# damien911224/ZeroShotVideoClassification

Hardware: AMD Instinct MI355X
Metric: clips/sec (fwd+bwd+step) R(2+1)D-18 16x112x112 bs=22/GPU (higher is better)
Workload: dtype f32

## Files before the change

### zeroshotvideoclassification_amd/csrc/conv_wgrad.hip

```cpp
#include <hip/hip_runtime.h>
#include <stdint.h>
#include <stdlib.h>
#include "conv_params.h"
#include "knobs.h"

namespace zsv {

typedef float f32x2 __attribute__((ext_vector_type(2)));

struct WgradParams {
    int M;
    int Cin, Cpad, nblk;
    int taps, kHW, kW;
    int Kp;
    int P;
    int oS, oHW, oW;
    Magic m_oS, m_oHW, m_oW;
    int gT, gH, gW, gS, gHW, gCS;
    int sT, sH, sW, pT, pH, pW;
    int chunks_per_slice;
    unsigned x_bytes, dy_bytes;
};

template <int TM, int TN, int WGM, int WGN, bool AV4, int BP, bool TWOTAP>
__global__ __launch_bounds__(256, (BP == 16 ? 3 : 2)) void conv_wgrad_kernel(WgradParams prm, const float* __restrict__ X,
                                                         const float* __restrict__ DY,
                                                         float* __restrict__ OUT, int tiles_m, int tiles_mn) {
    constexpr int BM = 16 * TM * WGM;
    constexpr int BN = 16 * TN * WGN;
    constexpr int LDK = BP + 2;
    constexpr int NBLK = BN / 16;
    constexpr int RW = 64 / BP;
    constexpr int RPP = 4 * RW;
    constexpr int PB = 16 / RPP;
    constexpr int BPASS = NBLK * PB;
    constexpr int AQ = BP / 4;
    constexpr int ARP = 256 / AQ;
    constexpr int APASS = AV4 ? (BM + ARP - 1) / ARP : BM / RPP;
    constexpr unsigned OOB = 0xFFFFFFFFu;
    static_assert(WGM * WGN == 4, "4 waves");
    static_assert(BM % RPP == 0 || AV4, "tile rows must be a multiple of the staging pass");

    __shared__ __attribute__((aligned(16))) float As[2][BM * LDK];
    __shared__ float Bs[2][BN * LDK];

    const int tid = threadIdx.x;
    const int lane = tid & 63;
    const int wave = sgpr(tid >> 6);
    const int wm0 = (wave / WGN) * (16 * TM);
    const int wn0 = (wave % WGN) * (16 * TN);
    const int lin = xcd_tile(gridDim.x, blockIdx.x);
    const int tile = lin % tiles_mn;
    const int slice = lin / tiles_mn;
    const int m0 = (tile % tiles_m) * BM;
    const int n0 = (tile / tiles_m) * BN;

    const __amdgpu_buffer_rsrc_t x_rsrc = __builtin_amdgcn_make_buffer_rsrc(const_cast<float*>(X), 0, prm.x_bytes, 0x00020000);
// ... 157 lines not shown
    const int frag_k = lane >> 4;
    const int frag_r = lane & 15;
    constexpr int NG = BP / 8;
    for (int ch = chunk_begin; ch < chunk_end; ++ch) {
        const int cur = (ch - chunk_begin) & 1;
        if (ch + 1 < chunk_end) store_chunk(cur ^ 1);
        const int lchunk = min(ch + 2, chunk_end - 1);
        const float* as = &As[cur][0];
        const float* bs = &Bs[cur][0];
        float a[2][2][TM], b[2][2][TN];
        auto fetch = [&](int g, int slot) {
#pragma unroll
            for (int kk = 0; kk < 2; ++kk) {
#pragma unroll
                for (int i = 0; i < TM; ++i) a[slot][kk][i] = as[(wm0 + 16 * i + frag_r) * LDK + (2 * g + kk) * 4 + frag_k];
#pragma unroll
                for (int j = 0; j < TN; ++j) b[slot][kk][j] = bs[(wn0 + 16 * j + frag_r) * LDK + (2 * g + kk) * 4 + frag_k];
            }
        };
        fetch(0, 0);
#pragma unroll
        for (int g = 0; g < NG; ++g) {
            if (g + 1 < NG) fetch(g + 1, (g + 1) & 1);
            __builtin_amdgcn_sched_barrier(0);
            load_part(lchunk, g, NG);
#pragma unroll
            for (int kk = 0; kk < 2; ++kk)
#pragma unroll
                for (int i = 0; i < TM; ++i)
#pragma unroll
                    for (int j = 0; j < TN; ++j)
                        acc[i][j] = __builtin_amdgcn_mfma_f32_16x16x4f32(a[g & 1][kk][i], b[g & 1][kk][j], acc[i][j], 0, 0, 0);
            __builtin_amdgcn_sched_barrier(0);
        }
        __syncthreads();
    }

    float* out = OUT + (size_t)slice * prm.M * prm.Kp;
#pragma unroll
    for (int j = 0; j < TN; ++j) {
        const int k = n0 + wn0 + 16 * j + frag_r;
        if (k >= prm.Kp) continue;
#pragma unroll
        for (int i = 0; i < TM; ++i) {
#pragma unroll
            for (int r = 0; r < 4; ++r) {
                const int m = m0 + wm0 + 16 * i + 4 * frag_k + r;
                if (m < prm.M) out[(size_t)m * prm.Kp + k] = acc[i][j][r];
            }
        }
    }
}

__global__ __launch_bounds__(256) void slab_sum_kernel(const float* __restrict__ slabs, float* __restrict__ out,
                                                       int M, int Cin, int taps, int Cpad, int slices) {
    __shared__ float part[8][32];
    const size_t slab = (size_t)M * taps * Cpad;
    const int e = threadIdx.x & 31, g = threadIdx.x >> 5;
    for (size_t j0 = (size_t)blockIdx.x * 32; j0 < slab; j0 += (size_t)gridDim.x * 32) {
        const size_t j = j0 + e;
        const int ci = (int)(j % Cpad);
        const bool live = j < slab && ci < Cin;
        float s = 0.f;
        if (live) {
            const float* src = slabs + j;
            int k = g;
            for (; k + 24 < slices; k += 32) {
                const float v0 = src[(size_t)k * slab], v1 = src[(size_t)(k + 8) * slab];
                const float v2 = src[(size_t)(k + 16) * slab], v3 = src[(size_t)(k + 24) * slab];
                s += v0; s += v1; s += v2; s += v3;
            }
            for (; k < slices; k += 8) s += src[(size_t)k * slab];
        }
        part[g][e] = s;
        __syncthreads();
        if (g == 0 && live) {
            float t = part[0][e];
#pragma unroll
            for (int q = 1; q < 8; ++q) t += part[q][e];
            const size_t r = j / Cpad;
            const int tap = (int)(r % taps);
            const int co = (int)(r / taps);
            out[((size_t)co * Cin + ci) * taps + tap] = t;
        }
        __syncthreads();
    }
}

__global__ __launch_bounds__(256) void slab_sum_rows_kernel(const float* __restrict__ slabs, float* __restrict__ out,
                                                            int M, int Cin, int taps, int Cpad, int slices) {
    extern __shared__ __attribute__((aligned(16))) float row[];
    const int co = blockIdx.x;
    const int len = taps * Cpad;
    const size_t slab = (size_t)M * len;
    const float* src = slabs + (size_t)co * len;
    for (int i = 4 * (int)threadIdx.x; i < len; i += 1024) {
        f32x4 t = *reinterpret_cast<const f32x4*>(src + i);
        int k = 1;
        for (; k + 2 < slices; k += 3) {
            const f32x4 v0 = *reinterpret_cast<const f32x4*>(src + (size_t)k * slab + i);
            const f32x4 v1 = *reinterpret_cast<const f32x4*>(src + (size_t)(k + 1) * slab + i);
            const f32x4 v2 = *reinterpret_cast<const f32x4*>(src + (size_t)(k + 2) * slab + i);
            t += v0; t += v1; t += v2;
        }
        for (; k < slices; ++k) t += *reinterpret_cast<const f32x4*>(src + (size_t)k * slab + i);
        *reinterpret_cast<f32x4*>(row + i) = t;
    }
    __syncthreads();
    float* dst = out + (size_t)co * Cin * taps;
    const int n = Cin * taps;
    for (int o = (int)threadIdx.x; o < n; o += 256) {
        const int ci = o / taps, tap = o - ci * taps;
        dst[o] = row[tap * Cpad + ci];
    }
}

int slab_sum(const float* slabs, float* dw, int M, int Cin, int taps, int Cpad, int slices, hipStream_t stream) {
    const size_t row_bytes = (size_t)taps * Cpad * sizeof(float);
    if (slices <= 32 && (long)M * slices <= 16384 && row_bytes <= 64 * 1024 && (reinterpret_cast<uintptr_t>(slabs) & 15) == 0 && !ZSV_KNOB(NO_SLAB_SUM_ROWS)) {
        static const hipError_t attr = hipFuncSetAttribute((const void*)slab_sum_rows_kernel, hipFuncAttributeMaxDynamicSharedMemorySize, 64 * 1024);
        if (attr != hipSuccess) return ZSV_E_LAUNCH;
        hipLaunchKernelGGL(slab_sum_rows_kernel, dim3((unsigned)M), dim3(256), row_bytes, stream, slabs, dw, M, Cin, taps, Cpad, slices);
        return hipGetLastError() == hipSuccess ? ZSV_OK : ZSV_E_LAUNCH;
    }
    const long n = (long)M * taps * Cpad;
    long blocks = (n + 31) / 32;
    if (blocks > 8192) blocks = 8192;
    hipLaunchKernelGGL(slab_sum_kernel, dim3((unsigned)blocks), dim3(256), 0, stream, slabs, dw, M, Cin, taps, Cpad, slices);
    return hipGetLastError() == hipSuccess ? ZSV_OK : ZSV_E_LAUNCH;
}

static int wgrad_bp() { return 32; }

__global__ __launch_bounds__(256) void t2_fold_kernel(const float* __restrict__ dw2, float* __restrict__ dw, int Cout, int Cin) {
    const long n = (long)Cout * Cin;
    for (long i = (long)blockIdx.x * 256 + threadIdx.x; i < n; i += (long)gridDim.x * 256) {
        const long co = i / Cin, c = i - co * Cin;
        const float* r0 = dw2 + (2 * co) * (2L * Cin) + 2 * c;
        const float* r1 = r0 + 2L * Cin;
        const f32x2 a = *reinterpret_cast<const f32x2*>(r0), b = *reinterpret_cast<const f32x2*>(r1);
        dw[3 * i] = b[0];
        dw[3 * i + 1] = a[0] + b[1];
        dw[3 * i + 2] = a[1];
    }
}

struct WgradPlan {
    int cfg;
    int bm, bn;
    int tiles_m, tiles_n, slices, chunks_per_slice;
    int Cpad, nblk, Kp;
};

static double wgrad_slices(long tiles, long chunks, int bp, int bm, int bn, long& slices) {
    const long lds_bytes = (long)(bm + bn) * 34 * 4 * 2;
    long per_cu = (160L * 1024) / lds_bytes;
    if (per_cu > 4) per_cu = 4;
    if (per_cu < 1) per_cu = 1;
    const long resident = 256L * per_cu;
    long max_slices = (chunks * bp + 511) / 512;
    if (max_slices < 1) max_slices = 1;
    if (max_slices > 1024) max_slices = 1024;
    slices = 1;
    double best_eff = -1.0;
    for (long s = 1; s <= max_slices && tiles * s <= 4 * resident + tiles; ++s) {
        const long wgs = tiles * s;
        const long rounds = (wgs + resident - 1) / resident;
        const double eff = (double)wgs / (double)(rounds * resident) - 0.02 * (double)wgs / (double)resident;
        if (eff > best_eff + 1e-9) { best_eff = eff; slices = s; }
    }
    return best_eff;
}

static WgradPlan wgrad_plan(const zsv_conv_desc* d) {
    WgradPlan pl;
    const int M = d->Cout;
    const int taps = d->kT * d->kH * d->kW;
    pl.nblk = (d->Cin + 15) / 16;
    pl.Cpad = pl.nblk * 16;
    pl.Kp = taps * pl.Cpad;
    const long P = (long)d->N * d->To * d->Ho * d->Wo;
    const int bp = wgrad_bp();
// ... 205 lines not shown
```

### zeroshotvideoclassification_amd/csrc/conv_wgrad_tring.hip

```cpp
#include <hip/hip_runtime.h>
#include <stdlib.h>

#include "conv_params.h"
#include "zsv_common.h"
#include "zsv_hip.h"
#include "knobs.h"

namespace zsv {

typedef __attribute__((address_space(3))) void* lds_ptr_t;

struct WgradTringParams {
    int M, Cin;
    int S, HW, T, nseg;
    int chunks_total, chunks_per_slice;
    int slices;
    unsigned x_bytes, dy_bytes;
    int tiles_m, tiles_mn;
    const float* pre_coef;
    int pre_pitch;
};

__device__ __forceinline__ int tring_swz(int row) { return ((row >> 2) & 1) << 1; }

template <int TM, bool PRE = false>
__global__ __launch_bounds__(256, 3) void conv_wgrad_tring_kernel(WgradTringParams prm, const float* __restrict__ X,
                                                                  const float* __restrict__ DY, float* __restrict__ OUT) {
#if defined(__HIP_DEVICE_COMPILE__)
    constexpr int BM = 16 * TM;
    constexpr int NAW = (TM + 3) / 4;
    constexpr int A_BYTES = TM * 1024;
    constexpr int RING_AT = 2 * A_BYTES;
    constexpr unsigned OOB = 0xFFFFFFF0u;
    extern __shared__ __attribute__((aligned(16))) unsigned char lds[];

    const int tid = threadIdx.x, lane = tid & 63;
    const int wave = __builtin_amdgcn_readfirstlane(tid >> 6);
    const int lid = xcd_tile(gridDim.x, blockIdx.x);
    const int tile = lid % prm.tiles_mn, slice = lid / prm.tiles_mn;
    const int m0 = (tile % prm.tiles_m) * BM, co0 = (tile / prm.tiles_m) * 64;
    const int c0 = slice * prm.chunks_per_slice;
    const int nq = min(prm.chunks_per_slice, prm.chunks_total - c0);
    if (nq <= 0) return;

    const __amdgpu_buffer_rsrc_t rs_x = __builtin_amdgcn_make_buffer_rsrc(const_cast<float*>(X), 0, prm.x_bytes, 0x00020000);
    const __amdgpu_buffer_rsrc_t rs_dy = __builtin_amdgcn_make_buffer_rsrc(const_cast<float*>(DY), 0, prm.dy_bytes, 0x00020000);

    const int prow = lane >> 2, srcslot = ((lane & 3) ^ tring_swz(prow)) * 4;
    int a_off[NAW];
#pragma unroll
    for (int k = 0; k < NAW; ++k) {
        const int pa = wave + 4 * k;
        const int ci = m0 + pa * 16 + prow;
        a_off[k] = (pa < TM && ci < prm.Cin) ? 4 * (ci * prm.S + srcslot) : -1;
    }
    const int co_l = co0 + wave * 16 + prow;
    const int b_off = co_l < prm.M ? 4 * (co_l * prm.S + srcslot) : -1;

    auto issue_x = [&](int buf, int n_img, int t, int seg) {
// ... 232 lines not shown
            const int sl = i & 1;
            if (i + 1 < TM) {
#pragma unroll
                for (int j = 0; j < 4; ++j) xf[sl ^ 1][j] = *reinterpret_cast<const f32x4*>(xs[j] + (i + 1) * 1024);
            }
            f32x4 d0 = xf[sl][0], d1 = xf[sl][1], d2 = xf[sl][2], d3 = xf[sl][3];
            if constexpr (PRE) {
#pragma unroll
                for (int s = 0; s < 4; ++s) {
                    d0[s] = fmaxf(__fmaf_rn(d0[s], pre_sc[i], pre_sh[i]), 0.f);
                    d1[s] = fmaxf(__fmaf_rn(d1[s], pre_sc[i], pre_sh[i]), 0.f);
                    d2[s] = fmaxf(__fmaf_rn(d2[s], pre_sc[i], pre_sh[i]), 0.f);
                    d3[s] = fmaxf(__fmaf_rn(d3[s], pre_sc[i], pre_sh[i]), 0.f);
                }
            }
            if (zero_d0) d0 = f32x4{0.f, 0.f, 0.f, 0.f};
            if (zero_d3) d3 = f32x4{0.f, 0.f, 0.f, 0.f};
            const f32x4 v0 = d0 - d2, v1 = d1 + d2, v2 = d2 - d1, v3 = d1 - d3;
            __builtin_amdgcn_sched_barrier(0);
            __builtin_amdgcn_s_setprio(1);
#pragma unroll
            for (int s = 0; s < 4; ++s) {
                acc[i][0] = __builtin_amdgcn_mfma_f32_16x16x4f32(v0[s], y0[s], acc[i][0], 0, 0, 0);
                acc[i][1] = __builtin_amdgcn_mfma_f32_16x16x4f32(v1[s], bsum[s], acc[i][1], 0, 0, 0);
                acc[i][2] = __builtin_amdgcn_mfma_f32_16x16x4f32(v2[s], bdif[s], acc[i][2], 0, 0, 0);
                acc[i][3] = __builtin_amdgcn_mfma_f32_16x16x4f32(v3[s], y1[s], acc[i][3], 0, 0, 0);
            }
            __builtin_amdgcn_s_setprio(0);
            __builtin_amdgcn_sched_barrier(0);
        }
        asm volatile("s_waitcnt vmcnt(0)" ::: "memory");
        __syncthreads();
        head = ring(head, 2);
        if (ntp == 0) job += prm.slices;
        tp = ntp; seg = nseg_; n_img = nn;
    }

    const int co = co0 + wave * 16 + r16;
    if (co < prm.M) {
        float* out = OUT + (size_t)slice * 4 * prm.Cin * prm.M;
#pragma unroll
        for (int p = 0; p < 4; ++p)
#pragma unroll
            for (int i = 0; i < TM; ++i)
#pragma unroll
                for (int r = 0; r < 4; ++r) {
                    const int ci = m0 + 16 * i + 4 * g + r;
                    if (ci < prm.Cin) out[((size_t)p * prm.Cin + ci) * prm.M + co] = acc[i][p][r];
                }
    }
#endif
}

__global__ __launch_bounds__(256) void wgrad_twino_sum_kernel(const float* __restrict__ slabs, float* __restrict__ dw, int M,
                                                              int Cin, int slices) {
    __shared__ float part[8][4][32];
    const size_t plane = (size_t)Cin * M;
    const int e = threadIdx.x & 31, grp = threadIdx.x >> 5;
    for (size_t j0 = (size_t)blockIdx.x * 32; j0 < plane; j0 += (size_t)gridDim.x * 32) {
        const size_t j = j0 + e;
        const bool live = j < plane;
        float s[4] = {0.f, 0.f, 0.f, 0.f};
        if (live) {
            int k = grp;
            for (; k + 24 < slices; k += 32) {
                float v[4][4];
#pragma unroll
                for (int u = 0; u < 4; ++u)
#pragma unroll
                    for (int p = 0; p < 4; ++p) v[u][p] = slabs[((size_t)(k + 8 * u) * 4 + p) * plane + j];
#pragma unroll
                for (int u = 0; u < 4; ++u)
#pragma unroll
                    for (int p = 0; p < 4; ++p) s[p] += v[u][p];
            }
            for (; k < slices; k += 8)
#pragma unroll
                for (int p = 0; p < 4; ++p) s[p] += slabs[((size_t)k * 4 + p) * plane + j];
        }
#pragma unroll
        for (int p = 0; p < 4; ++p) part[grp][p][e] = s[p];
        __syncthreads();
        if (grp == 0 && live) {
            float Mv[4];
#pragma unroll
            for (int p = 0; p < 4; ++p) {
                float t = part[0][p][e];
#pragma unroll
                for (int q = 1; q < 8; ++q) t += part[q][p][e];
                Mv[p] = t;
            }
            const int co = (int)(j % M), ci = (int)(j / M);
            float* o = dw + ((size_t)co * Cin + ci) * 3;
            const float h = 0.5f * (Mv[1] + Mv[2]);
            o[0] = Mv[0] + h;
            o[1] = 0.5f * (Mv[1] - Mv[2]);
            o[2] = h - Mv[3];
        }
        __syncthreads();
    }
}

__global__ __launch_bounds__(256) void wgrad_tring_sum_kernel(const float* __restrict__ slabs, float* __restrict__ dw, int M,
                                                              int Cin, int slices) {
    __shared__ float part[8][32];
    const size_t slab = (size_t)Cin * 3 * M;
    const int e = threadIdx.x & 31, grp = threadIdx.x >> 5;
    for (size_t j0 = (size_t)blockIdx.x * 32; j0 < slab; j0 += (size_t)gridDim.x * 32) {
        const size_t j = j0 + e;
        const bool live = j < slab;
        float s = 0.f;
        if (live) {
            int k = grp;
            for (; k + 24 < slices; k += 32) {
                const float v0 = slabs[(size_t)k * slab + j], v1 = slabs[(size_t)(k + 8) * slab + j];
                const float v2 = slabs[(size_t)(k + 16) * slab + j], v3 = slabs[(size_t)(k + 24) * slab + j];
                s += v0; s += v1; s += v2; s += v3;
            }
            for (; k < slices; k += 8) s += slabs[(size_t)k * slab + j];
        }
        part[grp][e] = s;
        __syncthreads();
        if (grp == 0 && live) {
            float v = part[0][e];
#pragma unroll
            for (int q = 1; q < 8; ++q) v += part[q][e];
            const int co = (int)(j % M);
            const size_t rr = j / M;
            const int kt = (int)(rr % 3), ci = (int)(rr / 3);
            dw[((size_t)co * Cin + ci) * 3 + kt] = v;
        }
        __syncthreads();
    }
}

struct WgradTringPlan {
    int tm, tiles_m, tiles_n, slices, chunks_per_slice;
};

static WgradTringPlan wgrad_tring_plan(const zsv_conv_desc* d) {
    WgradTringPlan pl;
    const int C = d->Cin;
    const int p9 = (C + 143) / 144 * 144, p8 = (C + 127) / 128 * 128;
    pl.tm = p9 <= p8 ? 9 : 8;
    const int bm = 16 * pl.tm;
    pl.tiles_m = (C + bm - 1) / bm;
    pl.tiles_n = (d->Cout + 63) / 64;
    const long chunks = (long)d->N * d->Ti * (d->Hi * d->Wi / 16);
    const long tiles = (long)pl.tiles_m * pl.tiles_n;
    long resident = pl.tm == 9 ? 512 : 768;
    if (const char* e = ZSV_KNOB(WGRAD_TRING_RESIDENT)) resident = atol(e) > 0 ? atol(e) : resident;
    const double t_mfma = 2.0 * (double)(pl.tiles_m * bm) * (double)(pl.tiles_n * 192) * (double)chunks * 16.0 / 1.1e14;
    const double t_slice = 2.0 * (double)C * 3.0 * d->Cout * sizeof(float) / 6.0e12;
    long max_sl = chunks / 32;
    if (max_sl < 1) max_sl = 1;
    if (max_sl > 4096) max_sl = 4096;
    long sl = 1;
    double best = 1e300;
    for (long c = 1; c <= max_sl; ++c) {
        const long wgs = tiles * c, rounds = (wgs + resident - 1) / resident;
        const double cost = t_mfma * (double)(rounds * resident) / (double)wgs + t_slice * (double)c;
        if (cost < best * 0.999) { best = cost; sl = c; }
    }
    if (const char* e = ZSV_KNOB(WGRAD_TRING_SLICES)) sl = atol(e) > 0 ? atol(e) : 1;
    if (sl > chunks) sl = chunks;
    pl.chunks_per_slice = (int)((chunks + sl - 1) / sl);
    pl.slices = (int)((chunks + pl.chunks_per_slice - 1) / pl.chunks_per_slice);
    return pl;
}

bool wgrad_tring_applicable(const zsv_conv_desc* d, const float* x, const float* dy) {
    if (ZSV_KNOB(NO_WGRAD_TRING)) return false;
    if (d->kT != 3 || d->kH != 1 || d->kW != 1 || d->sT != 1 || d->sH != 1 || d->sW != 1 || d->pT != 1 || d->pH != 0 || d->pW != 0)
        return false;
    if (d->Ti % 4 != 0 || (d->Hi * d->Wi) % 16 != 0) return false;
    if (d->Cout < 32) return false;
    const long S = (long)d->Ti * d->Hi * d->Wi;
    if ((long)d->N * d->Cin * S >= (1L << 29) || (long)d->N * d->Cout * S >= (1L << 29)) return false;
    const int C = d->Cin, p9 = (C + 143) / 144 * 144, p8 = (C + 127) / 128 * 128, pc = p9 <= p8 ? p9 : p8;
    if (pc * 10 > C * 13) return false;
    const int pm = (d->Cout + 63) / 64 * 64;
    if (pm * 10 > d->Cout * 13) return false;
    if ((long)d->N * S < 16384) return false;
    if (x != nullptr && ((reinterpret_cast<uintptr_t>(x) | reinterpret_cast<uintptr_t>(dy)) & 15) != 0) return false;
    return true;
}

// ... 43 lines not shown

template <int TM, bool PRE>
static int wgrad_twino_launch(const WgradTringParams& p, int slices, hipStream_t stream, const float* x, const float* dy,
                              float* out) {
    constexpr int LDS_BYTES = 6 * TM * 1024 + 4 * 4096;
    static const hipError_t attr = hipFuncSetAttribute((const void*)conv_wgrad_twino_kernel<TM, PRE>,
                                                       hipFuncAttributeMaxDynamicSharedMemorySize, LDS_BYTES);
    if (attr != hipSuccess) return ZSV_E_LAUNCH;
    hipLaunchKernelGGL((conv_wgrad_twino_kernel<TM, PRE>), dim3((unsigned)(p.tiles_mn * slices)), dim3(256), LDS_BYTES, stream, p, x,
                       dy, out);
    return launch_status();
}

template <int TM, bool PRE>
static int wgrad_tring_launch(const WgradTringParams& p, int slices, hipStream_t stream, const float* x, const float* dy,
                              float* out) {
    constexpr int LDS_BYTES = 2 * TM * 1024 + 4 * 4096;
    static const hipError_t attr = hipFuncSetAttribute((const void*)conv_wgrad_tring_kernel<TM, PRE>,
                                                       hipFuncAttributeMaxDynamicSharedMemorySize, LDS_BYTES);
    if (attr != hipSuccess) return ZSV_E_LAUNCH;
    hipLaunchKernelGGL((conv_wgrad_tring_kernel<TM, PRE>), dim3((unsigned)(p.tiles_mn * slices)), dim3(256), LDS_BYTES, stream, p, x,
                       dy, out);
    return launch_status();
}

int wgrad_tring(const zsv_conv_desc* d, const float* x, const float* dy, float* dw, void* workspace, size_t workspace_bytes,
                hipStream_t stream) {
    return wgrad_tring_pre(d, x, nullptr, 0, dy, dw, workspace, workspace_bytes, stream);
}

int wgrad_tring_pre(const zsv_conv_desc* d, const float* x, const float* pre_coef, int pre_pitch, const float* dy, float* dw,
                    void* workspace, size_t workspace_bytes, hipStream_t stream) {
    const bool twino = wgrad_twino_shape(d);
    const WgradTringPlan pl = twino ? wgrad_twino_plan(d) : wgrad_tring_plan(d);
    if (!workspace || workspace_bytes < wgrad_tring_workspace_bytes(d)) return ZSV_E_WORKSPACE;
    WgradTringParams p;
    p.M = d->Cout; p.Cin = d->Cin;
    p.S = d->Ti * d->Hi * d->Wi; p.HW = d->Hi * d->Wi; p.T = d->Ti; p.nseg = p.HW / 16;
    p.chunks_total = d->N * (twino ? p.T / 2 : p.T) * p.nseg;
    p.chunks_per_slice = pl.chunks_per_slice;
    p.slices = pl.slices;
    p.x_bytes = 4u * (unsigned)((long)d->N * d->Cin * p.S);
    p.dy_bytes = 4u * (unsigned)((long)d->N * d->Cout * p.S);
    p.tiles_m = pl.tiles_m; p.tiles_mn = pl.tiles_m * pl.tiles_n;
    p.pre_coef = pre_coef; p.pre_pitch = pre_pitch;
    float* slabs = (float*)workspace;
    int st;
    if (twino) {
        if (pre_coef) st = pl.tm == 9 ? wgrad_twino_launch<9, true>(p, pl.slices, stream, x, dy, slabs)
                                      : wgrad_twino_launch<8, true>(p, pl.slices, stream, x, dy, slabs);
        else st = pl.tm == 9 ? wgrad_twino_launch<9, false>(p, pl.slices, stream, x, dy, slabs)
                             : wgrad_twino_launch<8, false>(p, pl.slices, stream, x, dy, slabs);
        if (st) return st;
        const long n = (long)d->Cin * d->Cout;
        long blocks = (n + 31) / 32;
        if (blocks > 8192) blocks = 8192;
        hipLaunchKernelGGL(wgrad_twino_sum_kernel, dim3((unsigned)blocks), dim3(256), 0, stream, (const float*)slabs, dw, d->Cout,
                           d->Cin, pl.slices);
        return launch_status();
    }
    if (pre_coef) st = pl.tm == 9 ? wgrad_tring_launch<9, true>(p, pl.slices, stream, x, dy, slabs)
                                  : wgrad_tring_launch<8, true>(p, pl.slices, stream, x, dy, slabs);
    else st = pl.tm == 9 ? wgrad_tring_launch<9, false>(p, pl.slices, stream, x, dy, slabs)
                         : wgrad_tring_launch<8, false>(p, pl.slices, stream, x, dy, slabs);
    if (st) return st;
    const long n = (long)d->Cin * 3 * d->Cout;
    long blocks = (n + 31) / 32;
    if (blocks > 8192) blocks = 8192;
    hipLaunchKernelGGL(wgrad_tring_sum_kernel, dim3((unsigned)blocks), dim3(256), 0, stream, (const float*)slabs, dw, d->Cout,
                       d->Cin, pl.slices);
    return launch_status();
}

}
```

### zeroshotvideoclassification_amd/csrc/conv_wgrad_wino.hip

```cpp
#include <hip/hip_runtime.h>
#include <stdlib.h>

#include "conv_params.h"
#include "zsv_common.h"
#include "zsv_hip.h"
#include "knobs.h"

namespace zsv {

typedef __attribute__((address_space(3))) void* lds_ptr_t;
typedef unsigned u32x4w __attribute__((ext_vector_type(4)));

struct WgradWinoParams {
    int M, Cin, Cpad, R, Kp;
    int S, HW, W, kT;
    int chunks_total, chunks_per_slice, cpc;
    unsigned x_bytes, dy_bytes, vm_bytes;
    int tiles_m, tiles_mn;
};

template <int TM, int TN, bool EDGE>
__global__ __launch_bounds__(256, 2) void conv_wgrad_wino_kernel(WgradWinoParams prm, const float* __restrict__ X,
                                                                 const float* __restrict__ DY,
                                                                 const unsigned* __restrict__ VM, float* __restrict__ OUT) {
#if defined(__HIP_DEVICE_COMPILE__)
    constexpr int BM = 16 * TM;
    constexpr int LDA = 36, LDB = 44;
    constexpr int NA_TOT = (BM * 9 + 63) / 64;
    constexpr int BN = 64 * TN;
    constexpr int NB_TOT = 11 * TN;
    constexpr int NA = (NA_TOT + 3) / 4, NB = (NB_TOT + 3) / 4;
    constexpr int A_BYTES = NA_TOT * 1024, B_BYTES = NB_TOT * 1024;
    constexpr int VM_AT = A_BYTES + B_BYTES;
    constexpr int STAGE = VM_AT + 1024;
    constexpr unsigned OOB = 0xFFFFFFF0u;
    extern __shared__ __attribute__((aligned(16))) unsigned char lds[];

    const int tid = threadIdx.x, lane = tid & 63;
    const int wave = __builtin_amdgcn_readfirstlane(tid >> 6);
    const int lid = xcd_tile(gridDim.x, blockIdx.x);
    const int tile = lid % prm.tiles_mn, slice = lid / prm.tiles_mn;
    const int m0 = (tile % prm.tiles_m) * BM, n0 = (tile / prm.tiles_m) * BN;
    const int c0 = slice * prm.chunks_per_slice;
    const int nq = min(prm.chunks_per_slice, prm.chunks_total - c0);
    const int cpc = prm.cpc;
    int n_img = c0 / cpc;
    int p_local = (c0 - n_img * cpc) * 32;

    const __amdgpu_buffer_rsrc_t rs_dy = __builtin_amdgcn_make_buffer_rsrc(const_cast<float*>(DY), 0, prm.dy_bytes, 0x00020000);
    const __amdgpu_buffer_rsrc_t rs_x = __builtin_amdgcn_make_buffer_rsrc(const_cast<float*>(X), 0, prm.x_bytes, 0x00020000);
    const __amdgpu_buffer_rsrc_t rs_vm = __builtin_amdgcn_make_buffer_rsrc(const_cast<unsigned*>(VM), 0, prm.vm_bytes, 0x00020000);

    int a_off[NA], a_vox[NA];
#pragma unroll
    for (int k = 0; k < NA; ++k) {
        const int id = 64 * (wave + 4 * k) + lane;
        const int row = id / 9, pc = id - row * 9;
        const bool ok = row < BM && m0 + row < prm.M && pc < 8;
        a_off[k] = ok ? 4 * ((m0 + row) * prm.S + 4 * pc) : -1;
// ... 270 lines not shown
                V[4][s] = fmaf(-2.f, t5, t6);
                V[5][s] = fmaf(4.f, d1, fmaf(-5.f, d3, d5));
            }
        }
#pragma unroll
        for (int i = 0; i < TMX; ++i) {
            if (TMA != TMB && i >= tmw) break;
            const int sl = i & 1;
            if (i + 1 < TMX) {
                ar[sl ^ 1][0] = *reinterpret_cast<const f32x4*>(st + a_frag + (i + 1) * 16 * LDA * 4);
                ar[sl ^ 1][1] = *reinterpret_cast<const f32x4*>(st + a_frag + (i + 1) * 16 * LDA * 4 + 16);
            }
            float Av[6][2];
#pragma unroll
            for (int s = 0; s < 2; ++s) {
                const float y0 = ar[sl][s][0], y1 = ar[sl][s][1], y2 = ar[sl][s][2], y3 = ar[sl][s][3];
                const float e = y0 + y2, o = y1 + y3, e4 = fmaf(4.f, y2, y0), q = fmaf(4.f, y3, y1);
                Av[0][s] = y0; Av[1][s] = e + o; Av[2][s] = e - o;
                Av[3][s] = fmaf(2.f, q, e4); Av[4][s] = fmaf(-2.f, q, e4); Av[5][s] = y3;
            }
            __builtin_amdgcn_sched_barrier(0);
            __builtin_amdgcn_s_setprio(1);
#pragma unroll
            for (int s = 0; s < 2; ++s)
#pragma unroll
                for (int p = 0; p < 6; ++p)
                    acc[p][i] = __builtin_amdgcn_mfma_f32_16x16x4f32(Av[p][s], V[p][s], acc[p][i], 0, 0, 0);
            __builtin_amdgcn_s_setprio(0);
            __builtin_amdgcn_sched_barrier(0);
        }
        asm volatile("s_waitcnt vmcnt(0)" ::: "memory");
        __syncthreads();
    }

    float* out = OUT + (size_t)slice * 6 * prm.M * prm.Kp;
    const int n = n0 + 16 * cw + r16;
    if (n < prm.Kp) {
#pragma unroll
        for (int p = 0; p < 6; ++p)
#pragma unroll
            for (int i = 0; i < TMX; ++i) {
                if (TMA != TMB && i >= tmw) break;
#pragma unroll
                for (int r = 0; r < 4; ++r) {
                    const int m = m0 + 16 * (i0 + i) + 4 * g + r;
                    if (m < prm.M) out[((size_t)p * prm.M + m) * prm.Kp + n] = acc[p][i][r];
                }
            }
    }
#endif
}

template <int PTS>
__global__ __launch_bounds__(256) void wgrad_wino_sum_kernel(const float* __restrict__ slabs, float* __restrict__ dw, int M,
                                                             int Cin, int R, int Cpad, int slices) {
    __shared__ float part[8][PTS][32];
    const size_t plane = (size_t)M * R * Cpad;
    const int e = threadIdx.x & 31, grp = threadIdx.x >> 5;
    for (size_t j0 = (size_t)blockIdx.x * 32; j0 < plane; j0 += (size_t)gridDim.x * 32) {
        const size_t j = j0 + e;
        const int ci = (int)(j % Cpad);
        const bool live = j < plane && ci < Cin;
        float s[PTS];
#pragma unroll
        for (int p = 0; p < PTS; ++p) s[p] = 0.f;
        if (live) {
            int k = grp;
            for (; k + 8 < slices; k += 16) {
                float v[2][PTS];
#pragma unroll
                for (int u = 0; u < 2; ++u)
#pragma unroll
                    for (int p = 0; p < PTS; ++p) v[u][p] = slabs[((size_t)(k + 8 * u) * PTS + p) * plane + j];
#pragma unroll
                for (int u = 0; u < 2; ++u)
#pragma unroll
                    for (int p = 0; p < PTS; ++p) s[p] += v[u][p];
            }
            for (; k < slices; k += 8)
#pragma unroll
                for (int p = 0; p < PTS; ++p) s[p] += slabs[((size_t)k * PTS + p) * plane + j];
        }
#pragma unroll
        for (int p = 0; p < PTS; ++p) part[grp][p][e] = s[p];
        __syncthreads();
        if (grp == 0 && live) {
            float Mv[PTS];
#pragma unroll
            for (int p = 0; p < PTS; ++p) {
                float t = part[0][p][e];
#pragma unroll
                for (int q = 1; q < 8; ++q) t += part[q][p][e];
                Mv[p] = t;
            }
            const size_t rr = j / Cpad;
            const int r = (int)(rr % R), co = (int)(rr / R);
            float* o = dw + (((size_t)co * Cin + ci) * R + r) * 3;
            if constexpr (PTS == 4) {
                const float h = 0.5f * (Mv[1] + Mv[2]);
                o[0] = Mv[0] + h;
                o[1] = 0.5f * (Mv[1] - Mv[2]);
                o[2] = h - Mv[3];
            } else {
                const float s12 = Mv[1] + Mv[2], d12 = Mv[2] - Mv[1], s34 = Mv[3] + Mv[4], d34 = Mv[3] - Mv[4];
                o[0] = 0.25f * Mv[0] - s12 * (1.f / 6.f) + s34 * (1.f / 24.f);
                o[1] = d12 * (1.f / 6.f) + d34 * (1.f / 12.f);
                o[2] = Mv[5] - s12 * (1.f / 6.f) + s34 * (1.f / 6.f);
            }
        }
        __syncthreads();
    }
}

struct WgradWinoPlan {
    int tm, tn, tiles_m, tiles_n, slices, chunks_per_slice, Cpad, Kp;
};

static WgradWinoPlan wgrad_wino_plan(const zsv_conv_desc* d) {
    WgradWinoPlan pl;
    const int M = d->Cout;
    pl.Cpad = (d->Cin + 15) / 16 * 16;
    pl.Kp = 3 * d->kT * pl.Cpad;
    const int p9 = (M + 143) / 144 * 144, p8 = (M + 127) / 128 * 128;
    pl.tm = M <= 64 ? 4 : (p9 <= p8 ? 9 : 8);
    pl.tn = pl.tm == 4 ? 2 : 1;
    const int bm = 16 * pl.tm, bn = 64 * pl.tn;
    pl.tiles_m = (M + bm - 1) / bm;
    pl.tiles_n = (pl.Kp + bn - 1) / bn;
    const long chunks = (long)d->N * (((long)d->Ti * d->Hi * d->Wi + 31) / 32);
    const long tiles = (long)pl.tiles_m * pl.tiles_n, resident = 512;
    const double voxels = (double)chunks * 32.0;
    const double t_mfma = 4.0 * (double)(pl.tiles_m * bm) * (double)(pl.tiles_n * bn) * voxels / 1.1e14;
    const double t_slice = 2.0 * 4.0 * (double)M * pl.Kp * sizeof(float) / 6.0e12;
    long max_sl = chunks / 24;
    if (max_sl < 1) max_sl = 1;
    if (max_sl > 4096) max_sl = 4096;
    long sl = 1;
    double best = 1e300;
    for (long c = 1; c <= max_sl; ++c) {
        const long wgs = tiles * c, rounds = (wgs + resident - 1) / resident;
        const double cost = t_mfma * (double)(rounds * resident) / (double)wgs + t_slice * (double)c;
        if (cost < best * 0.999) { best = cost; sl = c; }
    }
    if (const char* e = ZSV_KNOB(WGRAD_WINO_SLICES)) sl = atol(e);
    if (sl < 1) sl = 1;
    if (sl > chunks) sl = chunks;
    pl.chunks_per_slice = (int)((chunks + sl - 1) / sl);
    pl.slices = (int)((chunks + pl.chunks_per_slice - 1) / pl.chunks_per_slice);
    return pl;
}

bool wgrad_wino_applicable(const zsv_conv_desc* d, const float* x, const float* dy) {
    if (ZSV_KNOB(NO_WINO) || ZSV_KNOB(NO_WGRAD_WINO)) return false;
    if ((d->kT != 1 && d->kT != 3) || d->kH != 3 || d->kW != 3 || d->sT != 1 || d->sH != 1 || d->sW != 1 || d->pT != d->kT / 2 ||
        d->pH != 1 || d->pW != 1)
        return false;
    if (d->Wi % 2 != 0 || d->Cin < 16) return false;
    const long S = (long)d->Ti * d->Hi * d->Wi;
    if (S % 4 != 0) return false;
    if ((long)d->N * d->Cin * S >= (1L << 29) || (long)d->N * d->Cout * S >= (1L << 29)) return false;
    const int M = d->Cout, p9 = (M + 143) / 144 * 144, p8 = (M + 127) / 128 * 128, pm = M <= 64 ? 64 : (p9 <= p8 ? p9 : p8);
    if (pm * 10 > M * 13) return false;
    if ((long)d->N * S < 16384) return false;
    if (x != nullptr && ((reinterpret_cast<uintptr_t>(x) | reinterpret_cast<uintptr_t>(dy)) & 15) != 0) return false;
    return true;
// ... 75 lines not shown
    constexpr int LDS_BYTES = 2 * (((16 * TM * 9 + 63) / 64 + 11 * TN + 1) * 1024);
    static const hipError_t attr = hipFuncSetAttribute((const void*)conv_wgrad_wino_kernel<TM, TN, EDGE>,
                                                       hipFuncAttributeMaxDynamicSharedMemorySize, LDS_BYTES);
    if (attr != hipSuccess) return ZSV_E_LAUNCH;
    hipLaunchKernelGGL((conv_wgrad_wino_kernel<TM, TN, EDGE>), dim3((unsigned)(p.tiles_mn * slices)), dim3(256), LDS_BYTES, stream, p, x,
                       dy, vm, out);
    return launch_status();
}

int wgrad_wino(const zsv_conv_desc* d, const float* x, const float* dy, float* dw, void* workspace, size_t workspace_bytes,
               hipStream_t stream, const unsigned* vm_ext) {
    const bool f43 = wgrad_wino4_applicable(d);
    WgradWinoPlan pl = wgrad_wino_plan(d);
    WgradWino4Plan p4{};
    if (f43) {
        p4 = wgrad_wino4_plan(d);
        pl.tiles_m = p4.tiles_m; pl.tiles_n = p4.tiles_n; pl.slices = p4.slices; pl.chunks_per_slice = p4.chunks_per_slice;
    }
    const int points = f43 ? 6 : 4;
    if (!workspace || workspace_bytes < wgrad_wino_workspace_bytes(d)) return ZSV_E_WORKSPACE;
    WgradWinoParams p;
    p.M = d->Cout; p.Cin = d->Cin; p.Cpad = pl.Cpad; p.R = 3 * d->kT; p.Kp = pl.Kp;
    p.S = d->Ti * d->Hi * d->Wi; p.HW = d->Hi * d->Wi; p.W = d->Wi; p.kT = d->kT;
    p.cpc = (p.S + 31) / 32;
    p.chunks_total = d->N * p.cpc;
    p.chunks_per_slice = pl.chunks_per_slice;
    p.x_bytes = 4u * (unsigned)((long)d->N * d->Cin * p.S);
    p.dy_bytes = 4u * (unsigned)((long)d->N * d->Cout * p.S);
    p.vm_bytes = 4u * (unsigned)p.S;
    p.tiles_m = pl.tiles_m; p.tiles_mn = pl.tiles_m * pl.tiles_n;
    float* slabs = (float*)workspace;
    const unsigned* vm = vm_ext;
    int st = ZSV_OK;
    if (vm == nullptr) {
        unsigned* own = (unsigned*)((char*)workspace + wgrad_wino_workspace_bytes(d) - (size_t)p.S * sizeof(unsigned));
        st = wgrad_vmask(d, own, stream);
        if (st) return st;
        vm = own;
    }
    const bool edge = p.S % 32 != 0 || d->Wi % 4 != 0;
    if (f43)
        st = p4.tma == 5 ? wgrad_wino4_launch<5, 4>(p, pl.slices, stream, x, dy, vm, slabs)
                         : wgrad_wino4_launch<4, 4>(p, pl.slices, stream, x, dy, vm, slabs);
    else if (pl.tm == 9)
        st = edge ? wgrad_wino_launch<9, 1, true>(p, pl.slices, stream, x, dy, vm, slabs)
                  : wgrad_wino_launch<9, 1, false>(p, pl.slices, stream, x, dy, vm, slabs);
    else if (pl.tm == 8)
        st = edge ? wgrad_wino_launch<8, 1, true>(p, pl.slices, stream, x, dy, vm, slabs)
                  : wgrad_wino_launch<8, 1, false>(p, pl.slices, stream, x, dy, vm, slabs);
    else
        st = edge ? wgrad_wino_launch<4, 2, true>(p, pl.slices, stream, x, dy, vm, slabs)
                  : wgrad_wino_launch<4, 2, false>(p, pl.slices, stream, x, dy, vm, slabs);
    if (st) return st;
    const long n = (long)d->Cout * p.R * pl.Cpad;
    long blocks = (n + 31) / 32;
    if (blocks > 8192) blocks = 8192;
    if (points == 6)
        hipLaunchKernelGGL(wgrad_wino_sum_kernel<6>, dim3((unsigned)blocks), dim3(256), 0, stream, (const float*)slabs, dw, d->Cout,
                           d->Cin, p.R, pl.Cpad, pl.slices);
    else
        hipLaunchKernelGGL(wgrad_wino_sum_kernel<4>, dim3((unsigned)blocks), dim3(256), 0, stream, (const float*)slabs, dw, d->Cout,
                           d->Cin, p.R, pl.Cpad, pl.slices);
    return launch_status();
}

}
```

Measured before the change: 573.2.

## Unify slab reduction kernels with vectorized multi-point loads and channel-split rows

Replaces the per-path slab-sum reduction kernels (plain, tring, twino, winograd) with one templated slab_sum_groups kernel. The new kernel loads f32x4 vectors when aligned, spreads Winograd points across lanes, and unrolls the slice loop more deeply to keep more loads in flight. The row-based slab sum also splits channels across a second grid dimension when there are few rows, pads the LDS pitch, and processes several items per thread. The goal is better memory bandwidth and occupancy in the wgrad reduction, at the cost of more template instantiations and more complex indexing.

Result: no change. 571.9 (-0.2%).

```diff
diff --git a/zeroshotvideoclassification_amd/csrc/conv_wgrad.hip b/zeroshotvideoclassification_amd/csrc/conv_wgrad.hip
--- a/zeroshotvideoclassification_amd/csrc/conv_wgrad.hip
+++ b/zeroshotvideoclassification_amd/csrc/conv_wgrad.hip
@@ -3,6 +3,7 @@
 #include <stdlib.h>
 #include "conv_params.h"
 #include "knobs.h"
+#include "slab_sum.h"
 
 namespace zsv {
 
@@ -266,82 +267,80 @@
     }
 }
 
-__global__ __launch_bounds__(256) void slab_sum_kernel(const float* __restrict__ slabs, float* __restrict__ out,
-                                                       int M, int Cin, int taps, int Cpad, int slices) {
-    __shared__ float part[8][32];
+struct SlabSumEpi {
+    float* out;
+    int Cin, taps, Cpad;
+    __device__ __forceinline__ bool live(size_t j) const { return (int)(j % Cpad) < Cin; }
+    __device__ __forceinline__ void store(size_t j, const float (&Mv)[1]) const {
+        const int ci = (int)(j % Cpad);
+        const size_t r = j / Cpad;
+        const int tap = (int)(r % taps);
+        const int co = (int)(r / taps);
+        out[((size_t)co * Cin + ci) * taps + tap] = Mv[0];
+    }
+};
+
+template <int IT>
+__global__ __launch_bounds__(256) void slab_sum_rows_kernel(const float* __restrict__ slabs, float* __restrict__ out,
+                                                            int M, int Cin, int taps, int Cpad, int slices, int cc, int pitch) {
+    extern __shared__ __attribute__((aligned(16))) float row[];
+    const int co = blockIdx.x, c0 = blockIdx.y * cc;
+    const int cw = Cpad - c0 < cc ? Cpad - c0 : cc;
+    const int qpt = cw / 4, items = taps * qpt;
     const size_t slab = (size_t)M * taps * Cpad;
-    const int e = threadIdx.x & 31, g = threadIdx.x >> 5;
-    for (size_t j0 = (size_t)blockIdx.x * 32; j0 < slab; j0 += (size_t)gridDim.x * 32) {
-        const size_t j = j0 + e;
-        const int ci = (int)(j % Cpad);
-        const bool live = j < slab && ci < Cin;
-        float s = 0.f;
-        if (live) {
-            const float* src = slabs + j;
-            int k = g;
-            for (; k + 24 < slices; k += 32) {
-                const float v0 = src[(size_t)k * slab], v1 = src[(size_t)(k + 8) * slab];
-                const float v2 = src[(size_t)(k + 16) * slab], v3 = src[(size_t)(k + 24) * slab];
-                s += v0; s += v1; s += v2; s += v3;
-            }
-            for (; k < slices; k += 8) s += src[(size_t)k * slab];
-        }
-        part[g][e] = s;
-        __syncthreads();
-        if (g == 0 && live) {
-            float t = part[0][e];
-#pragma unroll
-            for (int q = 1; q < 8; ++q) t += part[q][e];
-            const size_t r = j / Cpad;
-            const int tap = (int)(r % taps);
-            const int co = (int)(r / taps);
-            out[((size_t)co * Cin + ci) * taps + tap] = t;
-        }
-        __syncthreads();
-    }
-}
-
-__global__ __launch_bounds__(256) void slab_sum_rows_kernel(const float* __restrict__ slabs, float* __restrict__ out,
-                                                            int M, int Cin, int taps, int Cpad, int slices) {
-    extern __shared__ __attribute__((aligned(16))) float row[];
-    const int co = blockIdx.x;
-    const int len = taps * Cpad;
-    const size_t slab = (size_t)M * len;
-    const float* src = slabs + (size_t)co * len;
-    for (int i = 4 * (int)threadIdx.x; i < len; i += 1024) {
-        f32x4 t = *reinterpret_cast<const f32x4*>(src + i);
+    const float* base = slabs + (size_t)co * taps * Cpad + c0;
+    for (int it0 = (int)threadIdx.x; it0 < items; it0 += 256 * IT) {
+        const float* src[IT];
+        int dst[IT];
+#pragma unroll
+        for (int i = 0; i < IT; ++i) {
+            const int it = it0 + 256 * i < items ? it0 + 256 * i : it0;
+            const int tap = it / qpt, q = it - tap * qpt;
+            src[i] = base + tap * Cpad + 4 * q;
+            dst[i] = tap * pitch + 4 * q;
+        }
+        f32x4 t[IT];
+#pragma unroll
+        for (int i = 0; i < IT; ++i) t[i] = *reinterpret_cast<const f32x4*>(src[i]);
         int k = 1;
-        for (; k + 2 < slices; k += 3) {
-            const f32x4 v0 = *reinterpret_cast<const f32x4*>(src + (size_t)k * slab + i);
-            const f32x4 v1 = *reinterpret_cast<const f32x4*>(src + (size_t)(k + 1) * slab + i);
-            const f32x4 v2 = *reinterpret_cast<const f32x4*>(src + (size_t)(k + 2) * slab + i);
-            t += v0; t += v1; t += v2;
-        }
-        for (; k < slices; ++k) t += *reinterpret_cast<const f32x4*>(src + (size_t)k * slab + i);
-        *reinterpret_cast<f32x4*>(row + i) = t;
+        slab_chains<8 / IT>(t, src, slab, k, slices, 1);
+        if constexpr (8 / IT > 2) slab_chains<2>(t, src, slab, k, slices, 1);
+        slab_chains<1>(t, src, slab, k, slices, 1);
+#pragma unroll
+        for (int i = 0; i < IT; ++i)
+            if (i == 0 || it0 + 256 * i < items) *reinterpret_cast<f32x4*>(row + dst[i]) = t[i];
     }
     __syncthreads();
-    float* dst = out + (size_t)co * Cin * taps;
-    const int n = Cin * taps;
+    const int ce = (Cin < c0 + cw ? Cin : c0 + cw) - c0;
+    float* dstp = out + ((size_t)co * Cin + c0) * taps;
+    const int n = ce * taps;
     for (int o = (int)threadIdx.x; o < n; o += 256) {
         const int ci = o / taps, tap = o - ci * taps;
-        dst[o] = row[tap * Cpad + ci];
+        dstp[o] = row[tap * pitch + ci];
     }
 }
 
 int slab_sum(const float* slabs, float* dw, int M, int Cin, int taps, int Cpad, int slices, hipStream_t stream) {
     const size_t row_bytes = (size_t)taps * Cpad * sizeof(float);
     if (slices <= 32 && (long)M * slices <= 16384 && row_bytes <= 64 * 1024 && (reinterpret_cast<uintptr_t>(slabs) & 15) == 0 && !ZSV_KNOB(NO_SLAB_SUM_ROWS)) {
-        static const hipError_t attr = hipFuncSetAttribute((const void*)slab_sum_rows_kernel, hipFuncAttributeMaxDynamicSharedMemorySize, 64 * 1024);
-        if (attr != hipSuccess) return ZSV_E_LAUNCH;
-        hipLaunchKernelGGL(slab_sum_rows_kernel, dim3((unsigned)M), dim3(256), row_bytes, stream, slabs, dw, M, Cin, taps, Cpad, slices);
+        static const hipError_t attr[3] = {
+            hipFuncSetAttribute((const void*)slab_sum_rows_kernel<1>, hipFuncAttributeMaxDynamicSharedMemorySize, 64 * 1024),
+            hipFuncSetAttribute((const void*)slab_sum_rows_kernel<2>, hipFuncAttributeMaxDynamicSharedMemorySize, 64 * 1024),
+            hipFuncSetAttribute((const void*)slab_sum_rows_kernel<4>, hipFuncAttributeMaxDynamicSharedMemorySize, 64 * 1024)};
+        if (attr[0] != hipSuccess || attr[1] != hipSuccess || attr[2] != hipSuccess) return ZSV_E_LAUNCH;
+        int cc = Cpad;
+        while ((long)M * ((Cpad + cc - 1) / cc) < 512 && taps * (cc / 4) >= 512) cc = (cc / 2 + 15) / 16 * 16;
+        const int parts = (Cpad + cc - 1) / cc;
+        const int pitch = (size_t)taps * (cc + 4) * sizeof(float) <= 64 * 1024 ? cc + 4 : cc;
+        const int items = taps * (cc / 4);
+        const dim3 grid((unsigned)M, (unsigned)parts);
+        const size_t lds = (size_t)taps * pitch * sizeof(float);
+#define ZSV_ROWS(IT) hipLaunchKernelGGL(slab_sum_rows_kernel<IT>, grid, dim3(256), lds, stream, slabs, dw, M, Cin, taps, Cpad, slices, cc, pitch)
+        if (items <= 256) ZSV_ROWS(1); else if (items <= 512) ZSV_ROWS(2); else ZSV_ROWS(4);
+#undef ZSV_ROWS
         return hipGetLastError() == hipSuccess ? ZSV_OK : ZSV_E_LAUNCH;
     }
-    const long n = (long)M * taps * Cpad;
-    long blocks = (n + 31) / 32;
-    if (blocks > 8192) blocks = 8192;
-    hipLaunchKernelGGL(slab_sum_kernel, dim3((unsigned)blocks), dim3(256), 0, stream, slabs, dw, M, Cin, taps, Cpad, slices);
-    return hipGetLastError() == hipSuccess ? ZSV_OK : ZSV_E_LAUNCH;
+    return slab_sum_groups<1, 1>(slabs, (size_t)M * taps * Cpad, slices, SlabSumEpi{dw, Cin, taps, Cpad}, stream);
 }
 
 static int wgrad_bp() { return 32; }
diff --git a/zeroshotvideoclassification_amd/csrc/conv_wgrad_tring.hip b/zeroshotvideoclassification_amd/csrc/conv_wgrad_tring.hip
--- a/zeroshotvideoclassification_amd/csrc/conv_wgrad_tring.hip
+++ b/zeroshotvideoclassification_amd/csrc/conv_wgrad_tring.hip
@@ -5,6 +5,7 @@
 #include "zsv_common.h"
 #include "zsv_hip.h"
 #include "knobs.h"
+#include "slab_sum.h"
 
 namespace zsv {
 
@@ -343,87 +344,31 @@
 #endif
 }
 
-__global__ __launch_bounds__(256) void wgrad_twino_sum_kernel(const float* __restrict__ slabs, float* __restrict__ dw, int M,
-                                                              int Cin, int slices) {
-    __shared__ float part[8][4][32];
-    const size_t plane = (size_t)Cin * M;
-    const int e = threadIdx.x & 31, grp = threadIdx.x >> 5;
-    for (size_t j0 = (size_t)blockIdx.x * 32; j0 < plane; j0 += (size_t)gridDim.x * 32) {
-        const size_t j = j0 + e;
-        const bool live = j < plane;
-        float s[4] = {0.f, 0.f, 0.f, 0.f};
-        if (live) {
-            int k = grp;
-            for (; k + 24 < slices; k += 32) {
-                float v[4][4];
-#pragma unroll
-                for (int u = 0; u < 4; ++u)
-#pragma unroll
-                    for (int p = 0; p < 4; ++p) v[u][p] = slabs[((size_t)(k + 8 * u) * 4 + p) * plane + j];
-#pragma unroll
-                for (int u = 0; u < 4; ++u)
-#pragma unroll
-                    for (int p = 0; p < 4; ++p) s[p] += v[u][p];
-            }
-            for (; k < slices; k += 8)
-#pragma unroll
-                for (int p = 0; p < 4; ++p) s[p] += slabs[((size_t)k * 4 + p) * plane + j];
-        }
-#pragma unroll
-        for (int p = 0; p < 4; ++p) part[grp][p][e] = s[p];
-        __syncthreads();
-        if (grp == 0 && live) {
-            float Mv[4];
-#pragma unroll
-            for (int p = 0; p < 4; ++p) {
-                float t = part[0][p][e];
-#pragma unroll
-                for (int q = 1; q < 8; ++q) t += part[q][p][e];
-                Mv[p] = t;
-            }
-            const int co = (int)(j % M), ci = (int)(j / M);
-            float* o = dw + ((size_t)co * Cin + ci) * 3;
-            const float h = 0.5f * (Mv[1] + Mv[2]);
-            o[0] = Mv[0] + h;
-            o[1] = 0.5f * (Mv[1] - Mv[2]);
-            o[2] = h - Mv[3];
-        }
-        __syncthreads();
-    }
-}
-
-__global__ __launch_bounds__(256) void wgrad_tring_sum_kernel(const float* __restrict__ slabs, float* __restrict__ dw, int M,
-                                                              int Cin, int slices) {
-    __shared__ float part[8][32];
-    const size_t slab = (size_t)Cin * 3 * M;
-    const int e = threadIdx.x & 31, grp = threadIdx.x >> 5;
-    for (size_t j0 = (size_t)blockIdx.x * 32; j0 < slab; j0 += (size_t)gridDim.x * 32) {
-        const size_t j = j0 + e;
-        const bool live = j < slab;
-        float s = 0.f;
-        if (live) {
-            int k = grp;
-            for (; k + 24 < slices; k += 32) {
-                const float v0 = slabs[(size_t)k * slab + j], v1 = slabs[(size_t)(k + 8) * slab + j];
-                const float v2 = slabs[(size_t)(k + 16) * slab + j], v3 = slabs[(size_t)(k + 24) * slab + j];
-                s += v0; s += v1; s += v2; s += v3;
-            }
-            for (; k < slices; k += 8) s += slabs[(size_t)k * slab + j];
-        }
-        part[grp][e] = s;
-        __syncthreads();
-        if (grp == 0 && live) {
-            float v = part[0][e];
-#pragma unroll
-            for (int q = 1; q < 8; ++q) v += part[q][e];
-            const int co = (int)(j % M);
-            const size_t rr = j / M;
-            const int kt = (int)(rr % 3), ci = (int)(rr / 3);
-            dw[((size_t)co * Cin + ci) * 3 + kt] = v;
-        }
-        __syncthreads();
-    }
-}
+struct WgradTwinoSumEpi {
+    float* dw;
+    int M, Cin;
+    __device__ __forceinline__ bool live(size_t) const { return true; }
+    __device__ __forceinline__ void store(size_t j, const float (&Mv)[4]) const {
+        const int co = (int)(j % M), ci = (int)(j / M);
+        float* o = dw + ((size_t)co * Cin + ci) * 3;
+        const float h = 0.5f * (Mv[1] + Mv[2]);
+        o[0] = Mv[0] + h;
+        o[1] = 0.5f * (Mv[1] - Mv[2]);
+        o[2] = h - Mv[3];
+    }
+};
+
+struct WgradTringSumEpi {
+    float* dw;
+    int M, Cin;
+    __device__ __forceinline__ bool live(size_t) const { return true; }
+    __device__ __forceinline__ void store(size_t j, const float (&Mv)[1]) const {
+        const int co = (int)(j % M);
+        const size_t rr = j / M;
+        const int kt = (int)(rr % 3), ci = (int)(rr / 3);
+        dw[((size_t)co * Cin + ci) * 3 + kt] = Mv[0];
+    }
+};
 
 struct WgradTringPlan {
     int tm, tiles_m, tiles_n, slices, chunks_per_slice;
@@ -573,24 +518,14 @@
         else st = pl.tm == 9 ? wgrad_twino_launch<9, false>(p, pl.slices, stream, x, dy, slabs)
                              : wgrad_twino_launch<8, false>(p, pl.slices, stream, x, dy, slabs);
         if (st) return st;
-        const long n = (long)d->Cin * d->Cout;
-        long blocks = (n + 31) / 32;
-        if (blocks > 8192) blocks = 8192;
-        hipLaunchKernelGGL(wgrad_twino_sum_kernel, dim3((unsigned)blocks), dim3(256), 0, stream, (const float*)slabs, dw, d->Cout,
-                           d->Cin, pl.slices);
-        return launch_status();
+        return slab_sum_groups<4, 1>(slabs, (size_t)d->Cin * d->Cout, pl.slices, WgradTwinoSumEpi{dw, d->Cout, d->Cin}, stream);
     }
     if (pre_coef) st = pl.tm == 9 ? wgrad_tring_launch<9, true>(p, pl.slices, stream, x, dy, slabs)
                                   : wgrad_tring_launch<8, true>(p, pl.slices, stream, x, dy, slabs);
     else st = pl.tm == 9 ? wgrad_tring_launch<9, false>(p, pl.slices, stream, x, dy, slabs)
                          : wgrad_tring_launch<8, false>(p, pl.slices, stream, x, dy, slabs);
     if (st) return st;
-    const long n = (long)d->Cin * 3 * d->Cout;
-    long blocks = (n + 31) / 32;
-    if (blocks > 8192) blocks = 8192;
-    hipLaunchKernelGGL(wgrad_tring_sum_kernel, dim3((unsigned)blocks), dim3(256), 0, stream, (const float*)slabs, dw, d->Cout,
-                       d->Cin, pl.slices);
-    return launch_status();
-}
-
-}
+    return slab_sum_groups<1, 1>(slabs, (size_t)d->Cin * 3 * d->Cout, pl.slices, WgradTringSumEpi{dw, d->Cout, d->Cin}, stream);
+}
+
+}
diff --git a/zeroshotvideoclassification_amd/csrc/conv_wgrad_wino.hip b/zeroshotvideoclassification_amd/csrc/conv_wgrad_wino.hip
--- a/zeroshotvideoclassification_amd/csrc/conv_wgrad_wino.hip
+++ b/zeroshotvideoclassification_amd/csrc/conv_wgrad_wino.hip
@@ -5,6 +5,7 @@
 #include "zsv_common.h"
 #include "zsv_hip.h"
 #include "knobs.h"
+#include "slab_sum.h"
 
 namespace zsv {
 
@@ -381,65 +382,28 @@
 }
 
 template <int PTS>
-__global__ __launch_bounds__(256) void wgrad_wino_sum_kernel(const float* __restrict__ slabs, float* __restrict__ dw, int M,
-                                                             int Cin, int R, int Cpad, int slices) {
-    __shared__ float part[8][PTS][32];
-    const size_t plane = (size_t)M * R * Cpad;
-    const int e = threadIdx.x & 31, grp = threadIdx.x >> 5;
-    for (size_t j0 = (size_t)blockIdx.x * 32; j0 < plane; j0 += (size_t)gridDim.x * 32) {
-        const size_t j = j0 + e;
+struct WgradWinoSumEpi {
+    float* dw;
+    int Cin, R, Cpad;
+    __device__ __forceinline__ bool live(size_t j) const { return (int)(j % Cpad) < Cin; }
+    __device__ __forceinline__ void store(size_t j, const float (&Mv)[PTS]) const {
         const int ci = (int)(j % Cpad);
-        const bool live = j < plane && ci < Cin;
-        float s[PTS];
-#pragma unroll
-        for (int p = 0; p < PTS; ++p) s[p] = 0.f;
-        if (live) {
-            int k = grp;
-            for (; k + 8 < slices; k += 16) {
-                float v[2][PTS];
-#pragma unroll
-                for (int u = 0; u < 2; ++u)
-#pragma unroll
-                    for (int p = 0; p < PTS; ++p) v[u][p] = slabs[((size_t)(k + 8 * u) * PTS + p) * plane + j];
-#pragma unroll
-                for (int u = 0; u < 2; ++u)
-#pragma unroll
-                    for (int p = 0; p < PTS; ++p) s[p] += v[u][p];
-            }
-            for (; k < slices; k += 8)
-#pragma unroll
-                for (int p = 0; p < PTS; ++p) s[p] += slabs[((size_t)k * PTS + p) * plane + j];
+        const size_t rr = j / Cpad;
+        const int r = (int)(rr % R), co = (int)(rr / R);
+        float* o = dw + (((size_t)co * Cin + ci) * R + r) * 3;
+        if constexpr (PTS == 4) {
+            const float h = 0.5f * (Mv[1] + Mv[2]);
+            o[0] = Mv[0] + h;
+            o[1] = 0.5f * (Mv[1] - Mv[2]);
+            o[2] = h - Mv[3];
+        } else {
+            const float s12 = Mv[1] + Mv[2], d12 = Mv[2] - Mv[1], s34 = Mv[3] + Mv[4], d34 = Mv[3] - Mv[4];
+            o[0] = 0.25f * Mv[0] - s12 * (1.f / 6.f) + s34 * (1.f / 24.f);
+            o[1] = d12 * (1.f / 6.f) + d34 * (1.f / 12.f);
+            o[2] = Mv[5] - s12 * (1.f / 6.f) + s34 * (1.f / 6.f);
         }
-#pragma unroll
-        for (int p = 0; p < PTS; ++p) part[grp][p][e] = s[p];
-        __syncthreads();
-        if (grp == 0 && live) {
-            float Mv[PTS];
-#pragma unroll
-            for (int p = 0; p < PTS; ++p) {
-                float t = part[0][p][e];
-#pragma unroll
-                for (int q = 1; q < 8; ++q) t += part[q][p][e];
-                Mv[p] = t;
-            }
-            const size_t rr = j / Cpad;
-            const int r = (int)(rr % R), co = (int)(rr / R);
-            float* o = dw + (((size_t)co * Cin + ci) * R + r) * 3;
-            if constexpr (PTS == 4) {
-                const float h = 0.5f * (Mv[1] + Mv[2]);
-                o[0] = Mv[0] + h;
-                o[1] = 0.5f * (Mv[1] - Mv[2]);
-                o[2] = h - Mv[3];
-            } else {
-                const float s12 = Mv[1] + Mv[2], d12 = Mv[2] - Mv[1], s34 = Mv[3] + Mv[4], d34 = Mv[3] - Mv[4];
-                o[0] = 0.25f * Mv[0] - s12 * (1.f / 6.f) + s34 * (1.f / 24.f);
-                o[1] = d12 * (1.f / 6.f) + d34 * (1.f / 12.f);
-                o[2] = Mv[5] - s12 * (1.f / 6.f) + s34 * (1.f / 6.f);
-            }
-        }
-        __syncthreads();
-    }
-}
+    }
+};
 
 struct WgradWinoPlan {
     int tm, tn, tiles_m, tiles_n, slices, chunks_per_slice, Cpad, Kp;
@@ -621,16 +585,9 @@
         st = edge ? wgrad_wino_launch<4, 2, true>(p, pl.slices, stream, x, dy, vm, slabs)
                   : wgrad_wino_launch<4, 2, false>(p, pl.slices, stream, x, dy, vm, slabs);
     if (st) return st;
-    const long n = (long)d->Cout * p.R * pl.Cpad;
-    long blocks = (n + 31) / 32;
-    if (blocks > 8192) blocks = 8192;
-    if (points == 6)
-        hipLaunchKernelGGL(wgrad_wino_sum_kernel<6>, dim3((unsigned)blocks), dim3(256), 0, stream, (const float*)slabs, dw, d->Cout,
-                           d->Cin, p.R, pl.Cpad, pl.slices);
-    else
-        hipLaunchKernelGGL(wgrad_wino_sum_kernel<4>, dim3((unsigned)blocks), dim3(256), 0, stream, (const float*)slabs, dw, d->Cout,
-                           d->Cin, p.R, pl.Cpad, pl.slices);
-    return launch_status();
-}
-
-}
+    const size_t plane = (size_t)d->Cout * p.R * pl.Cpad;
+    if (points == 6) return slab_sum_groups<6, 3>(slabs, plane, pl.slices, WgradWinoSumEpi<6>{dw, d->Cin, p.R, pl.Cpad}, stream);
+    return slab_sum_groups<4, 1>(slabs, plane, pl.slices, WgradWinoSumEpi<4>{dw, d->Cin, p.R, pl.Cpad}, stream);
+}
+
+}
diff --git a/zeroshotvideoclassification_amd/csrc/slab_sum.h b/zeroshotvideoclassification_amd/csrc/slab_sum.h
--- /dev/null
+++ b/zeroshotvideoclassification_amd/csrc/slab_sum.h
@@ -0,0 +1,82 @@
+#pragma once
+#include <hip/hip_runtime.h>
+#include <stdint.h>
+#include "zsv_common.h"
+
+namespace zsv {
+
+template <int VEC> struct SlabVec { typedef float type; };
+template <> struct SlabVec<4> { typedef f32x4 type; };
+
+template <int U, int N, typename V>
+__device__ __forceinline__ void slab_chains(V (&s)[N], const float* (&src)[N], size_t stride, int& k, int kend, int step) {
+    for (; k + (U - 1) * step < kend; k += U * step) {
+        V v[U][N];
+#pragma unroll
+        for (int u = 0; u < U; ++u)
+#pragma unroll
+            for (int i = 0; i < N; ++i) v[u][i] = *reinterpret_cast<const V*>(src[i] + (size_t)(k + u * step) * stride);
+#pragma unroll
+        for (int u = 0; u < U; ++u)
+#pragma unroll
+            for (int i = 0; i < N; ++i) s[i] += v[u][i];
+    }
+}
+
+template <int PTS, int PPT, int VEC, class Epi>
+__global__ __launch_bounds__(256) void slab_sum_groups_kernel(const float* __restrict__ slabs, size_t plane, int slices, Epi epi) {
+    typedef typename SlabVec<VEC>::type V;
+    static_assert(PTS % PPT == 0 && 32 % (PTS / PPT) == 0, "point sets must tile the 32 lanes of a slice group");
+    constexpr int PS = PTS / PPT, QB = 32 / PS, EB = QB * VEC;
+    constexpr int U = PPT >= 3 ? 4 : 16 / PPT;
+    __shared__ __attribute__((aligned(16))) float part[8][PTS][EB];
+    const int lane = threadIdx.x & 31, grp = threadIdx.x >> 5;
+    const int q = lane % QB, p0 = (lane / QB) * PPT;
+    for (size_t j0 = (size_t)blockIdx.x * EB; j0 < plane; j0 += (size_t)gridDim.x * EB) {
+        const size_t j = j0 + (size_t)q * VEC;
+        V s[PPT];
+#pragma unroll
+        for (int i = 0; i < PPT; ++i) s[i] = V{};
+        if (j < plane && epi.live(j)) {
+            const float* src[PPT];
+#pragma unroll
+            for (int i = 0; i < PPT; ++i) src[i] = slabs + (size_t)(p0 + i) * plane + j;
+            int k = grp;
+            slab_chains<U>(s, src, (size_t)PTS * plane, k, slices, 8);
+            if constexpr (U > 4) slab_chains<4>(s, src, (size_t)PTS * plane, k, slices, 8);
+            slab_chains<1>(s, src, (size_t)PTS * plane, k, slices, 8);
+        }
+#pragma unroll
+        for (int i = 0; i < PPT; ++i) *reinterpret_cast<V*>(&part[grp][p0 + i][q * VEC]) = s[i];
+        __syncthreads();
+        const size_t je = j0 + threadIdx.x;
+        if (threadIdx.x < EB && je < plane && epi.live(je)) {
+            float Mv[PTS];
+#pragma unroll
+            for (int p = 0; p < PTS; ++p) {
+                float t = part[0][p][threadIdx.x];
+#pragma unroll
+                for (int g = 1; g < 8; ++g) t += part[g][p][threadIdx.x];
+                Mv[p] = t;
+            }
+            epi.store(je, Mv);
+        }
+        __syncthreads();
+    }
+}
+
+template <int PTS, int PPT, class Epi>
+static int slab_sum_groups(const float* slabs, size_t plane, int slices, const Epi& epi, hipStream_t stream) {
+    constexpr int QB = 32 / (PTS / PPT);
+    const bool vec = plane % 4 == 0 && (reinterpret_cast<uintptr_t>(slabs) & 15) == 0;
+    const size_t eb = (size_t)QB * (vec ? 4 : 1);
+    size_t blocks = (plane + eb - 1) / eb;
+    if (blocks > 8192) blocks = 8192;
+    if (vec)
+        hipLaunchKernelGGL((slab_sum_groups_kernel<PTS, PPT, 4, Epi>), dim3((unsigned)blocks), dim3(256), 0, stream, slabs, plane, slices, epi);
+    else
+        hipLaunchKernelGGL((slab_sum_groups_kernel<PTS, PPT, 1, Epi>), dim3((unsigned)blocks), dim3(256), 0, stream, slabs, plane, slices, epi);
+    return launch_status();
+}
+
+}
```
